# Evrytania/LTE-Cell-Scanner

Measured on NVIDIA H100. Metric: IQ Msamp/s through xcorr_pss, higher is better.
Workload: dtype s8 (3 exact int8 digits, int32 accumulate)

## Files before the change

lte-cell-scanner_b200/csrc/xcorr_tc.cu:

```cuda
#include <cstdio>
#include <cstdlib>
#include <cstring>
#include <cmath>

#include "lcs_ctx.hpp"
#include "wgmma_s8.hpp"

namespace lcs {

struct TcParams {
  const uint8_t* iq;
  unsigned long long iq_bytes;
  const uint32_t* buf_plan;
  const uint8_t* b_img;
  const float* corr;
  const tc::PassGeo* geo;
  const int16_t* dsh;
  float* single_planar;
  uint32_t n_cap, n_f_stride, n_comb, batch, n_pass;
  uint32_t tu, t_cta;
  uint32_t n_tiles_total;
  float inv2s;
  float rcp_ncomb;
};

__device__ __forceinline__ uint32_t smem_u32(const void* p) { return (uint32_t)__cvta_generic_to_shared(p); }
__device__ __forceinline__ void mbar_init(uint32_t bar, uint32_t count) {
  asm volatile("mbarrier.init.shared::cta.b64 [%0], %1;" ::"r"(bar), "r"(count));
}
__device__ __forceinline__ void mbar_arrive(uint32_t bar) {
  asm volatile("mbarrier.arrive.shared::cta.b64 _, [%0];" ::"r"(bar) : "memory");
}
__device__ __forceinline__ void mbar_arrive_expect_tx(uint32_t bar, uint32_t bytes) {
  asm volatile("mbarrier.arrive.expect_tx.shared::cta.b64 _, [%0], %1;" ::"r"(bar), "r"(bytes) : "memory");
}
#ifndef LCS_TC_WAIT_HINT_NS
#define LCS_TC_WAIT_HINT_NS 2000
#endif
__device__ __forceinline__ void mbar_wait(uint32_t bar, uint32_t parity) {
  asm volatile(
      "{\n"
      ".reg .pred p;\n"
      "WAIT_LOOP:\n"
      "mbarrier.try_wait.parity.shared::cta.b64 p, [%0], %1, %2;\n"
      "@p bra DONE;\n"
      "bra WAIT_LOOP;\n"
      "DONE:\n"
      "}\n" ::"r"(bar), "r"(parity), "r"(LCS_TC_WAIT_HINT_NS)
      : "memory");
}
__device__ __forceinline__ void bulk_g2s(uint32_t dst_smem, const void* src, uint32_t bytes, uint32_t bar) {
  asm volatile("cp.async.bulk.shared::cluster.global.mbarrier::complete_tx::bytes [%0], [%1], %2, [%3];" ::"r"(dst_smem), "l"(src),
               "r"(bytes), "r"(bar)
               : "memory");
}
__device__ __forceinline__ uint64_t make_desc(uint32_t saddr, uint32_t lbo_bytes, uint32_t sbo_bytes) {
  return (uint64_t)((saddr & 0x3FFFFu) >> 4) | ((uint64_t)(lbo_bytes >> 4) << 16) | ((uint64_t)(sbo_bytes >> 4) << 32);
}
__device__ __forceinline__ void wgmma_fence() { asm volatile("wgmma.fence.sync.aligned;" ::: "memory"); }
__device__ __forceinline__ void wgmma_commit() { asm volatile("wgmma.commit_group.sync.aligned;" ::: "memory"); }
template <int N>
__device__ __forceinline__ void wgmma_wait0(int (&d)[N]) {
  asm volatile("wgmma.wait_group.sync.aligned 0;" ::: "memory");
#pragma unroll
  for (int i = 0; i < N; i++) asm volatile("" : "+r"(d[i])::"memory");
}
__device__ __forceinline__ void fence_async_smem() { asm volatile("fence.proxy.async.shared::cta;" ::: "memory"); }
__device__ __forceinline__ void named_bar(uint32_t id, uint32_t nthreads) { asm volatile("bar.sync %0, %1;" ::"r"(id), "r"(nthreads) : "memory"); }

struct TcRun {
  uint32_t b, pp;
  int p0, p1;
  uint32_t n_tiles;
};
struct TcRunIter {
  uint32_t t, t_end;
  __device__ __forceinline__ void init(const TcParams& p) {
    t = blockIdx.x * p.t_cta;
    t_end = min(t + p.t_cta, p.n_tiles_total);
  }
  __device__ __forceinline__ bool next(const TcParams& p, TcRun& r) {
    while (t < t_end) {
      const uint32_t u = t / p.tu, base = u * p.tu, a = t - base;
      const uint32_t e = min(t_end, base + p.tu), bb = e - base;
      const uint32_t nb = (base + a) / p.t_cta - base / p.t_cta;
      t = e;
      const int p0 = 256 * (int)a - tc::HALO * (int)nb;
      if (p0 >= tc::N_FOLD) continue;
      int p1 = 256 * (int)bb - tc::HALO * (int)(nb + 1);
      if (p1 > tc::N_FOLD) p1 = tc::N_FOLD;
      r.p0 = p0;
      r.p1 = p1;
      r.n_tiles = min(bb - a, (uint32_t)(p1 - p0 + tc::HALO + tc::NT - 1) / tc::NT);
      if (p.buf_plan) {
        r.b = u / p.n_pass;
        r.pp = __ldg(p.buf_plan + r.b) * p.n_pass + (u - r.b * p.n_pass);
      } else {
        r.pp = u / p.batch;
        r.b = u - r.pp * p.batch;
      }
      return true;
    }
    return false;
  }
};
struct TcStep {
  TcRunIter it;
  TcRun r;
  uint32_t k, m;
  bool ok;
  __device__ __forceinline__ void init(const TcParams& p) { it.init(p); ok = it.next(p, r); k = 0; m = 0; }
  __device__ __forceinline__ void advance(const TcParams& p) {
    if (++m == p.n_comb) {
      m = 0;
      if (++k == r.n_tiles) { k = 0; ok = it.next(p, r); }
    }
  }
};

template <int C, int J>
struct TcSmem {
  static constexpr tc::Layout L{C, J};
  static constexpr int P = 0;
  static constexpr int B = P + 4 * tc::P_BYTES;
  static constexpr int WIN = B + L.b_bytes();
  static constexpr int CORR = WIN + L.npad() * tc::WROW * 4;
  static constexpr int DOFF = CORR + 2 * L.npad() * 4;
  static constexpr int RAW = DOFF + tc::M_MAX * L.npad() * 4;
  static constexpr int BAR = RAW + 2 * tc::RAW_BYTES;
  static constexpr int TOTAL = BAR + 8 * 8;
};

template <int C, int J>
__global__ void __launch_bounds__(128 + 128 * J, 1) xcorr_fold_tc_kernel(const __grid_constant__ TcParams p) {
  using SM = TcSmem<C, J>;
  constexpr tc::Layout LAY{C, J};
  constexpr int NPAD = LAY.npad(), NJOB = LAY.njob();
  constexpr int NACC = NJOB / 2;
  constexpr int CG = C / 8;
  constexpr int NV = C / 2;
  static_assert(C % 8 == 0, "digit planes must start on an 8-column group of the accumulator fragment");
  static_assert(SM::TOTAL <= 232448, "shared memory");
  extern __shared__ __align__(128) uint8_t smem[];
  const int tid = threadIdx.x, warp = tid >> 5, lane = tid & 31;
  uint8_t* sP = smem + SM::P;
  float* sWin = reinterpret_cast<float*>(smem + SM::WIN);
  float* sCorr = reinterpret_cast<float*>(smem + SM::CORR);
  int* sDoff = reinterpret_cast<int*>(smem + SM::DOFF);
  const uint32_t bar0 = smem_u32(smem + SM::BAR);
  const uint32_t BAR_PFULL = bar0, BAR_PEMPTY = bar0 + 16, BAR_RAW = bar0 + 32, BAR_BFULL = bar0 + 48;

  for (int i = tid; i < NPAD * tc::WROW; i += LAY.threads()) sWin[i] = 0.f;
  if (tid == 0) {
    for (int i = 0; i < 2; i++) {
      mbar_init(BAR_PFULL + 8 * i, 1);
      mbar_init(BAR_PEMPTY + 8 * i, 4 * J);
      mbar_init(BAR_RAW + 8 * i, 1);
      mbar_init(BAR_BFULL + 8 * i, 1);
    }
    asm volatile("fence.mbarrier_init.release.cluster;" ::: "memory");
  }
  __syncthreads();

  if (warp == 0) {
    const uint64_t iq_lo = reinterpret_cast<uint64_t>(p.iq), iq_hi = iq_lo + p.iq_bytes;
    const uint32_t raw_addr = smem_u32(smem + SM::RAW);
    auto issue_raw = [&](const TcStep& s, uint32_t rs) -> uint32_t {
      const int smin = __ldg(&p.geo[s.r.pp].smin[s.m]);
      const uint64_t z = iq_lo + 2ull * ((uint64_t)s.r.b * p.n_cap + (uint64_t)(s.r.p0 + (int)(tc::NT * s.k) + smin));
      const uint64_t zal = z & ~15ull;
      uint32_t bytes = 0, rem = 0;
      if (zal < iq_hi) {
        const uint64_t avail = iq_hi - zal;
        const uint64_t left = avail & ~15ull;
        if (left < (uint64_t)(tc::RAW_BYTES - 16)) { bytes = (uint32_t)left; rem = (uint32_t)(avail - left); }
        else bytes = (uint32_t)(tc::RAW_BYTES - 16);
      }
      if ((uint32_t)lane < rem) smem[SM::RAW + rs * tc::RAW_BYTES + bytes + lane] = __ldg(reinterpret_cast<const uint8_t*>(zal) + bytes + lane);
      if (lane == 0) {
        if (bytes) {
          mbar_arrive_expect_tx(BAR_RAW + 8 * rs, bytes);
          bulk_g2s(raw_addr + rs * tc::RAW_BYTES, reinterpret_cast<const void*>(zal), bytes, BAR_RAW + 8 * rs);
        } else {
          mbar_arrive(BAR_RAW + 8 * rs);
        }
      }
      return (uint32_t)(z - zal);
    };
    TcStep cur, nxt;
    cur.init(p);
    nxt = cur;
    if (nxt.ok) nxt.advance(p);
    uint32_t zo_cur = 0, zo_nxt = 0;
    if (cur.ok) zo_cur = issue_raw(cur, 0);
    for (uint32_t i = 0; cur.ok; i++) {
      const uint32_t stage = i & 1, use = i >> 1;
      if (nxt.ok) zo_nxt = issue_raw(nxt, stage ^ 1);
      mbar_wait(BAR_RAW + 8 * stage, use & 1);
      mbar_wait(BAR_PEMPTY + 8 * stage, (use & 1) ^ 1);
      const uint32_t* rw = reinterpret_cast<const uint32_t*>(smem + SM::RAW + stage * tc::RAW_BYTES);
      const int zo = (int)zo_cur;
      uint4* P1 = reinterpret_cast<uint4*>(sP + (stage * 2 + 0) * tc::P_BYTES);
      uint4* P2 = reinterpret_cast<uint4*>(sP + (stage * 2 + 1) * tc::P_BYTES);
#pragma unroll 2
      for (int row = lane; row < tc::NBLK * 8; row += 32) {
        const int o = zo + 16 * (row >> 3) + 2 * (row & 7);
        const int ow = o >> 2;
        const bool sh = (o & 3) != 0;
        uint32_t w[5];
#pragma unroll
        for (int e = 0; e < 5; e++) w[e] = rw[ow + e];
        uint32_t x[4], y[4];
#pragma unroll
        for (int e = 0; e < 4; e++) {
          const uint32_t v = sh ? __byte_perm(w[e], w[e + 1], 0x5432) : w[e];
          x[e] = v ^ 0x80808080u;
          y[e] = __byte_perm(v, 0, 0x2301) ^ 0x7F807F80u;
        }
        P1[row] = make_uint4(x[0], x[1], x[2], x[3]);
        P2[row] = make_uint4(y[0], y[1], y[2], y[3]);
      }
      __syncwarp();
      fence_async_smem();
      __syncwarp();
      if (lane == 0) mbar_arrive(BAR_PFULL + 8 * stage);
      cur = nxt;
      zo_cur = zo_nxt;
      if (nxt.ok) nxt.advance(p);
    }
  } else if (warp >= 4) {
    const int job = (warp >> 2) - 1;
    const int wq = warp & 3;
    const int wt = tid - 128 * (job + 1);
    const int cb = 2 * (lane & 3);
    const uint32_t BAR_ID = 1 + job;
    const uint32_t sP_addr = smem_u32(sP), sBj_addr = smem_u32(smem + SM::B + job * LAY.b_job_bytes());
    const uint32_t my_bfull = BAR_BFULL + 8 * job;
    char* myWinB = reinterpret_cast<char*>(sWin + (job * C + cb) * tc::WROW + tc::HALO + 16 * wq + (lane >> 2));
    const float* cre = sCorr + job * C + cb;
    const float* cim = sCorr + NPAD + job * C + cb;
    uint32_t cur_pp = 0xffffffffu, bfull_par = 0, step = 0;
    auto mma_part = [&](int (&acc)[NACC], uint32_t a_addr) {
      const uint64_t a_desc = make_desc(a_addr, 128, 128), b_desc = make_desc(sBj_addr, 128, tc::B_SBO);
      wgmma_fence();
#pragma unroll
      for (int s = 0; s < tc::KSTEPS; s++) tc::wgmma_s8<NJOB>(acc, a_desc + (uint64_t)(s * 16), b_desc + (uint64_t)(s * 16), s > 0);
      wgmma_commit();
      wgmma_wait0(acc);
    };
    auto recombine = [&](const int (&acc)[NACC], float (&x)[NV], const float* kc) {
#pragma unroll
      for (int g = 0; g < CG; g++) {
        const float2 k2 = *reinterpret_cast<const float2*>(kc + 8 * g);
        const float kk[2] = {k2.x, k2.y};
#pragma unroll
        for (int h = 0; h < 2; h++)
#pragma unroll
          for (int e = 0; e < 2; e++) {
            const int r = 4 * g + 2 * h + e;
            const int t = acc[r] * 256 + acc[r + 4 * CG];
            const float f2 = __int_as_float((int)tc::MAGIC_BITS + acc[r + 8 * CG]);
            x[(g * 2 + h) * 2 + e] = __fadd_rn(__fmaf_rn((float)t, 256.f, f2), kk[e]);
          }
      }
    };
    TcRunIter it;
    it.init(p);
    TcRun r;
    while (it.next(p, r)) {
      if (r.pp != cur_pp) {
        named_bar(BAR_ID, 128);
        if (wt == 0) {
          constexpr uint32_t B_BYTES = (uint32_t)LAY.b_job_bytes(), CHUNK = 27648;
          mbar_arrive_expect_tx(my_bfull, B_BYTES);
          const uint8_t* src = p.b_img + (size_t)r.pp * LAY.b_bytes() + (size_t)job * B_BYTES;
          for (uint32_t o = 0; o < B_BYTES; o += CHUNK) bulk_g2s(sBj_addr + o, src + o, min(CHUNK, B_BYTES - o), my_bfull);
        }
        const float* gc = p.corr + (size_t)r.pp * 2 * NPAD;
        const int16_t* gd = p.dsh + (size_t)r.pp * tc::M_MAX * NPAD;
        for (int i = wt; i < 2 * C; i += 128) {
          const int o = (i / C) * NPAD + job * C + i % C;
          sCorr[o] = __ldg(gc + o);
        }
        for (int i = wt; i < (int)p.n_comb * C; i += 128) {
          const int o = (i / C) * NPAD + job * C + i % C;
          sDoff[o] = -4 * (int)__ldg(gd + o);
        }
        named_bar(BAR_ID, 128);
        mbar_wait(my_bfull, bfull_par);
        bfull_par ^= 1;
        cur_pp = r.pp;
      }
      const int f0 = __ldg(&p.geo[r.pp].f0);
      const uint32_t n_templ = 3u * (uint32_t)__ldg(&p.geo[r.pp].n_f);
      for (uint32_t k = 0; k < r.n_tiles; k++) {
        for (uint32_t m = 0; m < p.n_comb; m++, step++) {
          const uint32_t stage = step & 1, use = step >> 1;
          int d[CG][2];
#pragma unroll
          for (int g = 0; g < CG; g++) {
            const int2 d2 = *reinterpret_cast<const int2*>(sDoff + m * NPAD + job * C + cb + 8 * g);
            d[g][0] = d2.x;
            d[g][1] = d2.y;
          }
          mbar_wait(BAR_PFULL + 8 * stage, use & 1);
          const uint32_t a_stage = sP_addr + stage * 2 * tc::P_BYTES;
#pragma unroll 1
          for (int q = 0; q < tc::NSUB; q++) {
            int acc[NACC];
            float x[NV], rr[NV];
            mma_part(acc, a_stage + q * (tc::NSUBL / 8) * 128);
            recombine(acc, x, cre);
#pragma unroll
            for (int v = 0; v < NV; v++) rr[v] = __fmul_rn(x[v], x[v]);
            mma_part(acc, a_stage + tc::P_BYTES + q * (tc::NSUBL / 8) * 128);
            if (q == tc::NSUB - 1 && lane == 0) mbar_arrive(BAR_PEMPTY + 8 * stage);
            recombine(acc, x, cim);
#pragma unroll
            for (int v = 0; v < NV; v++) rr[v] = __fmaf_rn(x[v], x[v], rr[v]);
#pragma unroll
            for (int g = 0; g < CG; g++)
#pragma unroll
              for (int h = 0; h < 2; h++)
#pragma unroll
                for (int e = 0; e < 2; e++)
                  x[(g * 2 + h) * 2 + e] =
                      *reinterpret_cast<const float*>(myWinB + d[g][e] + ((8 * g + e) * tc::WROW + q * tc::NSUBL + 8 * h) * 4);
#pragma unroll
            for (int g = 0; g < CG; g++)
#pragma unroll
              for (int h = 0; h < 2; h++)
#pragma unroll
                for (int e = 0; e < 2; e++) {
                  const int v = (g * 2 + h) * 2 + e;
                  *reinterpret_cast<float*>(myWinB + d[g][e] + ((8 * g + e) * tc::WROW + q * tc::NSUBL + 8 * h) * 4) = __fadd_rn(x[v], rr[v]);
                }
          }
          named_bar(BAR_ID, 128);
        }
        const float ncf = (float)p.n_comb, rcp = p.rcp_ncomb;
        const int pb = r.p0 + (int)(tc::NT * k) - tc::HALO;
        const bool last = k + 1 == r.n_tiles;
        const uint32_t row_end = min(n_templ, (uint32_t)((job + 1) * C));
        for (uint32_t row = job * C + wq; row < row_end; row += 4) {
          const uint32_t rf = row / 3, rt = row - 3 * rf;
          float* dst = p.single_planar + (((size_t)r.b * 3 + rt) * p.n_f_stride + f0 + rf) * tc::N_FOLD;
          float* src = sWin + row * tc::WROW;
#pragma unroll
          for (int j = lane; j < tc::NT; j += 32) {
            const int pos = pb + j;
            const float v = src[j];
            if (pos >= r.p0 && pos < r.p1) {
              const float x = __fmul_rn(v, p.inv2s);
              float qv;
              if (rcp != 0.f) {
                qv = __fmul_rn(x, rcp);
                qv = __fmaf_rn(__fmaf_rn(-ncf, qv, x), rcp, qv);
              } else {
                qv = __fdiv_rn(x, ncf);
              }
              dst[pos] = qv;
            }
          }
          const float carry = last ? 0.f : src[tc::NT + lane];
          __syncwarp();
          src[lane] = carry;
#pragma unroll
          for (int j = tc::HALO + lane; j < tc::WSTR; j += 32) src[j] = 0.f;
        }
        named_bar(BAR_ID, 128);
      }
    }
  }
}

template <int C, int J>
static cudaError_t tc_set_smem() {
  return cudaFuncSetAttribute(xcorr_fold_tc_kernel<C, J>, cudaFuncAttributeMaxDynamicSharedMemorySize, TcSmem<C, J>::TOTAL);
}
lcs_status tc_init(lcs_ctx* ctx) {
  LCS_CUDA(ctx, (tc_set_smem<16, 1>()));
  LCS_CUDA(ctx, (tc_set_smem<24, 2>()));
  LCS_CUDA(ctx, (tc_set_smem<32, 2>()));
  LCS_CUDA(ctx, (tc_set_smem<48, 2>()));
  return LCS_OK;
}

int launch_xcorr_fold_tc(PlanSet& ps, const void* d_iq_cu8, uint32_t batch, const uint32_t* d_buf_plan, float* d_single_planar,
                         cudaStream_t st) {
  const XcorrGeom& g = ps.geom;
  TcParams q;
  q.iq = reinterpret_cast<const uint8_t*>(d_iq_cu8);
  q.iq_bytes = (unsigned long long)batch * g.n_cap * 2;
  q.buf_plan = d_buf_plan;
  q.b_img = ps.d_b.p;
  q.corr = ps.d_corr.p;
  q.geo = ps.d_geo.p;
  q.dsh = ps.d_dsh.p;
  q.single_planar = d_single_planar;
  q.n_cap = g.n_cap;
  q.n_f_stride = g.n_f_stride;
  q.n_comb = g.n_comb_xc;
  q.batch = batch;
  q.n_pass = ps.n_pass;
  q.inv2s = ps.inv_scale * ps.inv_scale;
  static const bool kExactRcp[25] = {false, true, true, true, true, true, false, true, true, true, false, true, false,
                                     true, false, true, true, true, false, true, false, true, false, true, false};
  q.rcp_ncomb = (g.n_comb_xc <= 24 && kExactRcp[g.n_comb_xc]) ? 1.0f / (float)g.n_comb_xc : 0.f;
  const uint32_t n_units = batch * ps.n_pass, n_sm = (uint32_t)ps.ctx->n_sm;
  uint32_t tu = (tc::N_FOLD + tc::HALO + tc::NT - 1) / tc::NT, t_cta = 1;
  for (;; tu++) {
    t_cta = (uint32_t)(((uint64_t)n_units * tu + n_sm - 1) / n_sm);
    const uint32_t runs = (tu + t_cta - 1) / t_cta + 1;
    if ((int)(tc::NT * tu) - (int)(tc::HALO * runs) >= tc::N_FOLD) break;
  }
  q.tu = tu;
  q.t_cta = t_cta;
  q.n_tiles_total = n_units * tu;
  const uint32_t grid = (q.n_tiles_total + t_cta - 1) / t_cta;
  const tc::Layout& L = ps.lay;
  if (L.cj == 16) xcorr_fold_tc_kernel<16, 1><<<grid, L.threads(), TcSmem<16, 1>::TOTAL, st>>>(q);
  else if (L.cj == 24) xcorr_fold_tc_kernel<24, 2><<<grid, L.threads(), TcSmem<24, 2>::TOTAL, st>>>(q);
  else if (L.cj == 32) xcorr_fold_tc_kernel<32, 2><<<grid, L.threads(), TcSmem<32, 2>::TOTAL, st>>>(q);
  else xcorr_fold_tc_kernel<48, 2><<<grid, L.threads(), TcSmem<48, 2>::TOTAL, st>>>(q);
  return 1;
}

}
```

Measured before the change: 4383.

## Double-buffer wgmma accumulators and rebalance registers between producer and consumer warps

Splits the single accumulator into separate real and imaginary accumulators so the next wgmma group is issued before waiting on the previous one. Recombination and window updates can then overlap with tensor-core work instead of waiting on each group to finish. It also adds setmaxnreg so producer warps give up registers and consumer warpgroups gain them, and the sub-tile loop is fully unrolled. Idle producer warps 1-3 now return early. The risks are higher register pressure from two live accumulators and the full unroll, possible spills, and fragile wgmma wait ordering.

```diff
diff --git a/lte-cell-scanner_b200/csrc/xcorr_tc.cu b/lte-cell-scanner_b200/csrc/xcorr_tc.cu
--- a/lte-cell-scanner_b200/csrc/xcorr_tc.cu
+++ b/lte-cell-scanner_b200/csrc/xcorr_tc.cu
@@ -59,12 +59,16 @@
 }
 __device__ __forceinline__ void wgmma_fence() { asm volatile("wgmma.fence.sync.aligned;" ::: "memory"); }
 __device__ __forceinline__ void wgmma_commit() { asm volatile("wgmma.commit_group.sync.aligned;" ::: "memory"); }
-template <int N>
-__device__ __forceinline__ void wgmma_wait0(int (&d)[N]) {
-  asm volatile("wgmma.wait_group.sync.aligned 0;" ::: "memory");
+template <int PENDING, int N>
+__device__ __forceinline__ void wgmma_wait(int (&d)[N]) {
+  asm volatile("wgmma.wait_group.sync.aligned %0;" ::"n"(PENDING) : "memory");
 #pragma unroll
   for (int i = 0; i < N; i++) asm volatile("" : "+r"(d[i])::"memory");
 }
+template <uint32_t R>
+__device__ __forceinline__ void setmaxnreg_dec() { asm volatile("setmaxnreg.dec.sync.aligned.u32 %0;" ::"n"(R)); }
+template <uint32_t R>
+__device__ __forceinline__ void setmaxnreg_inc() { asm volatile("setmaxnreg.inc.sync.aligned.u32 %0;" ::"n"(R)); }
 __device__ __forceinline__ void fence_async_smem() { asm volatile("fence.proxy.async.shared::cta;" ::: "memory"); }
 __device__ __forceinline__ void named_bar(uint32_t id, uint32_t nthreads) { asm volatile("bar.sync %0, %1;" ::"r"(id), "r"(nthreads) : "memory"); }
 
@@ -141,6 +145,8 @@
   constexpr int NV = C / 2;
   static_assert(C % 8 == 0, "digit planes must start on an 8-column group of the accumulator fragment");
   static_assert(SM::TOTAL <= 232448, "shared memory");
+  constexpr uint32_t PROD_REGS = 40, CONS_REGS = J == 2 ? 232 : 240;
+  static_assert(128 * PROD_REGS + 128 * J * CONS_REGS <= 65536, "register file");
   extern __shared__ __align__(128) uint8_t smem[];
   const int tid = threadIdx.x, warp = tid >> 5, lane = tid & 31;
   uint8_t* sP = smem + SM::P;
@@ -162,7 +168,9 @@
   }
   __syncthreads();
 
-  if (warp == 0) {
+  if (warp < 4) {
+    setmaxnreg_dec<PROD_REGS>();
+    if (warp != 0) return;
     const uint64_t iq_lo = reinterpret_cast<uint64_t>(p.iq), iq_hi = iq_lo + p.iq_bytes;
     const uint32_t raw_addr = smem_u32(smem + SM::RAW);
     auto issue_raw = [&](const TcStep& s, uint32_t rs) -> uint32_t {
@@ -228,7 +236,8 @@
       zo_cur = zo_nxt;
       if (nxt.ok) nxt.advance(p);
     }
-  } else if (warp >= 4) {
+  } else {
+    setmaxnreg_inc<CONS_REGS>();
     const int job = (warp >> 2) - 1;
     const int wq = warp & 3;
     const int wt = tid - 128 * (job + 1);
@@ -246,8 +255,8 @@
 #pragma unroll
       for (int s = 0; s < tc::KSTEPS; s++) tc::wgmma_s8<NJOB>(acc, a_desc + (uint64_t)(s * 16), b_desc + (uint64_t)(s * 16), s > 0);
       wgmma_commit();
-      wgmma_wait0(acc);
     };
+    int acc_re[NACC], acc_im[NACC];
     auto recombine = [&](const int (&acc)[NACC], float (&x)[NV], const float* kc) {
 #pragma unroll
       for (int g = 0; g < CG; g++) {
@@ -296,28 +305,34 @@
       for (uint32_t k = 0; k < r.n_tiles; k++) {
         for (uint32_t m = 0; m < p.n_comb; m++, step++) {
           const uint32_t stage = step & 1, use = step >> 1;
-          int d[CG][2];
-#pragma unroll
-          for (int g = 0; g < CG; g++) {
-            const int2 d2 = *reinterpret_cast<const int2*>(sDoff + m * NPAD + job * C + cb + 8 * g);
-            d[g][0] = d2.x;
-            d[g][1] = d2.y;
-          }
           mbar_wait(BAR_PFULL + 8 * stage, use & 1);
           const uint32_t a_stage = sP_addr + stage * 2 * tc::P_BYTES;
-#pragma unroll 1
+          mma_part(acc_re, a_stage);
+#pragma unroll
           for (int q = 0; q < tc::NSUB; q++) {
-            int acc[NACC];
             float x[NV], rr[NV];
-            mma_part(acc, a_stage + q * (tc::NSUBL / 8) * 128);
-            recombine(acc, x, cre);
+            mma_part(acc_im, a_stage + tc::P_BYTES + q * (tc::NSUBL / 8) * 128);
+            wgmma_wait<1>(acc_re);
+            recombine(acc_re, x, cre);
 #pragma unroll
             for (int v = 0; v < NV; v++) rr[v] = __fmul_rn(x[v], x[v]);
-            mma_part(acc, a_stage + tc::P_BYTES + q * (tc::NSUBL / 8) * 128);
-            if (q == tc::NSUB - 1 && lane == 0) mbar_arrive(BAR_PEMPTY + 8 * stage);
-            recombine(acc, x, cim);
+            if (q + 1 < tc::NSUB) {
+              mma_part(acc_re, a_stage + (q + 1) * (tc::NSUBL / 8) * 128);
+              wgmma_wait<1>(acc_im);
+            } else {
+              wgmma_wait<0>(acc_im);
+              if (lane == 0) mbar_arrive(BAR_PEMPTY + 8 * stage);
+            }
+            recombine(acc_im, x, cim);
 #pragma unroll
             for (int v = 0; v < NV; v++) rr[v] = __fmaf_rn(x[v], x[v], rr[v]);
+            int d[CG][2];
+#pragma unroll
+            for (int g = 0; g < CG; g++) {
+              const int2 d2 = *reinterpret_cast<const int2*>(sDoff + m * NPAD + job * C + cb + 8 * g);
+              d[g][0] = d2.x;
+              d[g][1] = d2.y;
+            }
 #pragma unroll
             for (int g = 0; g < CG; g++)
 #pragma unroll
```

Result: faster. 4611, median of 6 (+5.2%).
